# drnatebrown/col-bwt

Measured on AMD Instinct MI355X. Metric: query bases/s, higher is better.
Workload: dtype int64

## Files before the change

col-bwt_amd/csrc/fat2_query.hip:

```cpp
#include <hip/hip_runtime.h>
#include <stdint.h>

#include "device_layout.h"
#include "fat_cursor.h"
#include "fat_layout.h"
#include "lane_io.h"
#include "lane_out.h"
#include "query_kernels.h"

namespace colbwt {

namespace {

constexpr uint32_t kOffMis0 = 0xFFFFFFFCu;
constexpr uint32_t kOffMis1 = 0xFFFFFFFBu;

#ifdef COLBWT_COUNT_TRIPS
#define FAT2_STAT(k) (++stat[k])
#else
#define FAT2_STAT(k) ((void)0)
#endif

__device__ __forceinline__ uint32_t mis_slot(const uint8_t *top, uint32_t own, uint32_t c) {
    const uint32_t aidx = top[own], cidx = top[c];
    const uint32_t slot = cidx < aidx ? cidx : cidx - 1;
    return cidx < 4 && slot < kFatSlots ? slot : kFatSlots;
}

template <int K, typename PmlT, bool kDeep>
__global__ __launch_bounds__(kQueryBlock)
void fat2_query_kernel(FatTable T, const uint8_t *__restrict__ bases, const uint64_t *__restrict__ read_off,
                       uint64_t n_reads, uint32_t big_reads, uint32_t tail_permille,
                       PmlT *__restrict__ pml, uint8_t *__restrict__ cid) {
    constexpr bool kWide = sizeof(PmlT) == 4;
    __shared__ uint4 s_stage[kWaves][8][64];
    __shared__ uint4 s_win[kWaves][4][64];
    __shared__ uint32_t s_claim;
    __shared__ uint8_t s_top[256];
    const uint32_t wave = threadIdx.x >> 6, lane = threadIdx.x & 63u, g8 = lane & ~7u, p = lane & 7u;
    uint32_t *const s_jx = reinterpret_cast<uint32_t *>(&s_stage[wave][7][48]);
    ChunkPlan plan;
    plan.init(n_reads, big_reads, tail_permille);
    if (threadIdx.x == 0) s_claim = 0;
    s_top[threadIdx.x] = (uint8_t)fat_top_index(T.top4, threadIdx.x);
    __syncthreads();
    uint32_t *const claim = &s_claim;
    ReadCursor rc;
    bool done;
    rc.c_next = threadIdx.x;
    rc.request_chunk(plan, read_off);
    rc.commit();
    done = !rc.enter_chunk(plan, claim);

    OutRuns acc;
    uint32_t trip = 0;
    LaneWindow win;
    win.init(rc.off + rc.k - 1);
    uint4 (*const my_win)[64] = s_win[wave];

    uint32_t j = done ? 0u : T.r - 1;
    uint32_t o = kOffLastPos;
    uint32_t L = 0;
    const uint4 *const my_row = &s_stage[wave][p][g8];

#ifdef COLBWT_COUNT_TRIPS
    unsigned long long stat[8] = {0, 0, 0, 0, 0, 0, 0, 0};
#endif
    while (__any(!done)) {
        bool step_back = false;
        if (!done && rc.k == 0 && !rc.next_in_flight && (rc.r != rc.r_lo || rc.nc_ready)) {
            if (rc.r != rc.r_lo) {
                rc.r -= 1;
                rc.k = rc.off - rc.next_off;
                rc.off = rc.next_off;
                step_back = rc.r > rc.r_lo;
            } else if (kWide || acc.cnt == 0) {
                done = !rc.enter_chunk(plan, claim);
                if (!done) win.init(rc.off + rc.k - 1);
            }
            j = done ? 0u : T.r - 1;
            o = kOffLastPos;
            L = 0;
        }
        const bool live = !done && rc.k != 0;
        uint64_t &k = rc.k;
        const uint64_t g = rc.off + k - 1;

        s_jx[lane] = j;
        wave_sync();
        {
            const uint4 ja = *reinterpret_cast<const uint4 *>(&s_jx[g8]);
            const uint4 jb = *reinterpret_cast<const uint4 *>(&s_jx[g8 + 4]);
            const uint32_t jq[8] = {ja.x, ja.y, ja.z, ja.w, jb.x, jb.y, jb.z, jb.w};
            wave_sync();
#pragma unroll
            for (uint32_t q = 0; q < 8; ++q)
                __builtin_amdgcn_global_load_lds(T.lines + (uint64_t)jq[q] * kFatRowBytes + ((p ^ q) << 4), &s_stage[wave][q][0],
                                                 16, 0, 0);
        }
        if (live && win.avail(g) < (k < 8u ? (uint32_t)k : 8u)) win.request(my_win, bases, g);
        if (step_back) { rc.in_next = read_off[rc.r - 1]; rc.next_in_flight = true; }
        if (!done && rc.fetch_pending) rc.request_chunk(plan, read_off);
        lds_dma_landed();
        rc.commit();

        const uint32_t have = live ? win.avail(g) : 0u;
        uint32_t consumed = 0, l_new = 0, keep = 0xFFFFFFFFu, keep1 = 0xFFFFFFFFu;
        uint64_t ids = 0;
        if (!live || have == 0) FAT2_STAT(5);
        if (live && have != 0) {
            const uint64_t W = win.get8(my_win, lane, g);
            const uint32_t left = k < have ? (uint32_t)k : have;
            if (o == kOffMis0 || o == kOffMis1) {
                FAT2_STAT(2);
                const uint32_t h4 = !kDeep && o == kOffMis1 ? 4u : 0u;
                const uint4 e0 = my_row[(h4 + 0u) ^ p], e1 = my_row[(h4 + 1u) ^ p], e2 = my_row[(h4 + 2u) ^ p],
                            e3 = my_row[(h4 + 3u) ^ p];
                const uint32_t carry = L;
                const uint32_t t1 = (e0.y >> 16) & 0xFFu, d1 = e0.y >> 24, v1 = e3.z & 7u;
                uint32_t oc = 4;
                if (left >= 2) {
                    const uint32_t c2 = (uint32_t)(W >> 48) & 0xFFu;
                    const uint32_t s2 = mis_slot(s_top, t1, c2);
                    if (c2 == t1) oc = 0;
                    else if (s2 < kFatSlots && ((v1 >> s2) & 1u)) oc = 1 + s2;
                }
                if (oc < 4) {
                    const uint32_t J = oc == 0 ? e0.z : oc == 1 ? e0.w : oc == 2 ? e1.x : e1.y;
                    const uint32_t rho = oc == 0 ? e1.z : oc == 1 ? e1.w : oc == 2 ? e2.x : e2.y;
                    const uint32_t pw = oc < 2 ? e2.z : e2.w, P = (oc & 1u) ? pw >> 16 : pw & 0xFFFFu;
                    const uint32_t ch = (e3.x >> (8 * oc)) & 0xFFu, cd = (e3.y >> (8 * oc)) & 0xFFu;
                    const uint32_t vo = (e3.z >> (4 + 4 * oc)) & 7u;
                    consumed = 2;
                    l_new = 1;
                    keep = oc == 0 ? 0xFFFFFFFFu : 0u;
                    ids = (uint64_t)(d1 | (carry << 8));
                    L = oc == 0 ? 1u : 0u;
                    uint32_t nJ = J, nP = P, nrho = rho, nch = ch, ncd = cd, nv = vo, seen = 2;
                    if constexpr (kDeep) {
                        if (left >= 3 && ((uint32_t)(W >> 40) & 0xFFu) == ch) {
                            const uint4 f0 = my_row[4u ^ p], f1 = my_row[5u ^ p], f2 = my_row[6u ^ p], f3 = my_row[7u ^ p];
                            nJ = oc == 0 ? f0.x : oc == 1 ? f0.y : oc == 2 ? f0.z : f0.w;
                            nrho = oc == 0 ? f1.x : oc == 1 ? f1.y : oc == 2 ? f1.z : f1.w;
                            const uint32_t pw2 = oc < 2 ? f2.x : f2.y;
                            nP = (oc & 1u) ? pw2 >> 16 : pw2 & 0xFFFFu;
                            nch = (f2.z >> (8 * oc)) & 0xFFu;
                            ncd = (f2.w >> (8 * oc)) & 0xFFu;
                            nv = (f3.x >> (4 * oc)) & 7u;
                            consumed = 3;
                            seen = 3;
                            ids = (uint64_t)(cd | (d1 << 8) | (carry << 16));
                            if (oc == 0) { l_new = 2; keep = 0xFFFFFFFFu; }
                            else { l_new = 1; keep = 0xFFFFFFFFu; keep1 = 0u; }
                            L += 1;
                        }
                    }
                    if (k > consumed) {
                        uint32_t sn = kFatSlots;
                        if (left > seen) {
                            const uint32_t cn = (uint32_t)(W >> (8u * (7u - seen))) & 0xFFu;
                            if (cn != nch) sn = mis_slot(s_top, nch, cn);
                        }
                        if (sn < kFatSlots && ((nv >> sn) & 1u)) {
                            const uint32_t e = nrho * kFatSlots + sn;
                            j = T.slot_line0 + (kDeep ? e : e >> 1);
                            o = kDeep ? kOffMis0 : kOffMis0 - (e & 1u);
                            L = ncd;
                        } else {
                            j = nJ;
                            o = nP;
                        }
                    }
                } else {
                    consumed = 1;
                    l_new = 0;
                    ids = (uint64_t)carry;
                    L = 0;
                    j = e0.x;
                    o = e0.y & 0xFFFFu;
                }
            } else {
                FAT2_STAT(0);
                const uint4 r0 = my_row[0 ^ p];
                const uint4 r1 = my_row[1 ^ p];
                const uint64_t CH = (uint64_t)r0.x | ((uint64_t)r0.y << 32);
                const uint64_t CID = (uint64_t)r0.z | ((uint64_t)r0.w << 32);
                const uint32_t len = r1.x & 0xFFFFu;
                uint32_t skip = 0;
                bool stay = false;
                if (o == kOffPred) { o = len - 1; skip = 1; }
                else if (o == kOffSucc) { o = 0; skip = 1; }
                else if (o >= len && j < T.r - 1) {
                    o -= len;
                    j += 1;
                    stay = true;
                    FAT2_STAT(1);
                } else {
                    o = o < len ? o : len - 1;
                }
                if (!stay) {
                    const uint64_t X = skip ? ((W >> 8) ^ CH) & 0x00FFFFFFFFFFFFFFull : W ^ CH;
                    const uint32_t run = matching_top_bytes(X);
                    const uint32_t cap = left + skip < (uint32_t)K ? left + skip : (uint32_t)K;
                    uint32_t steps = run < cap ? run : cap;
                    bool own_jump = true, to_entry = false;
                    uint32_t e_next = 0, carry = 0;
                    if (run < cap) {
                        const uint32_t d = run + 1u, sh = 8u * (8u - d);
                        const uint32_t c = (uint32_t)(W >> (sh + 8u * skip)) & 0xFFu;
                        const uint32_t s = mis_slot(s_top, (uint32_t)(CH >> sh) & 0xFFu, c);
                        if (s < kFatSlots && ((r1.w >> (3u * run + s)) & 1u)) {
                            const uint32_t rho = reinterpret_cast<const uint32_t *>(&my_row[((kFatRho / 16) + (run >> 2)) ^ p])[run & 3u];
                            e_next = rho * kFatSlots + s;
                            carry = (uint32_t)(CID >> sh) & 0xFFu;
                            to_entry = true;
                            own_jump = false;
                        }
                    }
                    if (run == 0 && !to_entry) {
                        const uint32_t c = (uint32_t)(W >> 56);
                        const uint32_t cidx = T.cmap[c];
                        bool moved = false;
                        if (cidx != kAbsent) moved = fat_threshold_scan(T, j, o, c, cidx);
                        FAT2_STAT(moved ? 3 : 4);
                        if (moved) {
                            steps = 1;
                            consumed = 1;
                            l_new = 0;
                            own_jump = false;
                        } else {
                            const uint32_t st = matching_top_bytes(X & 0x00FFFFFFFFFFFFFFull);
                            const uint32_t cap0 = left < (uint32_t)K ? left : (uint32_t)K;
                            steps = st < cap0 ? st : cap0;
                            consumed = steps;
                            l_new = steps - 1;
                        }
                    } else {
                        consumed = steps - skip;
                        l_new = L + consumed;
                    }
                    L = l_new;
                    ids = steps ? CID >> (8u * (8u - steps)) : 0ull;
                    if (k == consumed) {
                    } else if (to_entry) {
                        FAT2_STAT(6);
                        j = T.slot_line0 + (kDeep ? e_next : e_next >> 1);
                        o = kDeep ? kOffMis0 : kOffMis0 - (e_next & 1u);
                        L = carry;
                    } else if (own_jump) {
                        const uint32_t e = steps - 1;
                        const uint32_t I = reinterpret_cast<const uint32_t *>(&my_row[((kFatI / 16) + (e >> 2)) ^ p])[e & 3u];
                        const uint32_t Oh = reinterpret_cast<const uint16_t *>(&my_row[((kFatO / 16) + (e >> 3)) ^ p])[e & 7u];
                        const uint64_t cuts = (uint64_t)r1.y | ((uint64_t)r1.z << 32);
                        const uint32_t cut = (uint32_t)(cuts >> (8 * e)) & 0xFFu, cut_a = cut & 0xFu, len_b = cut >> 4;
                        j = I;
                        if (cut_a != kSKCutNone && o >= cut_a) {
                            j += 1;
                            o -= cut_a;
                            if (len_b != kSKCutNone && o >= len_b) {
                                j += 1;
                                o -= len_b;
                            }
                        } else {
                            o += Oh;
                        }
                    }
                }
            }
            if constexpr (kWide) {
                for (uint32_t e = 0; e < consumed; ++e) {
                    pml[g - consumed + 1 + e] = (PmlT)((e < 2 ? keep : keep1) ? l_new - e : 0u);
                    cid[g - consumed + 1 + e] = (uint8_t)(ids >> (8 * e));
                }
            } else {
                acc.push_run(consumed, l_new, keep, keep1, (uint32_t)ids, (uint32_t)(ids >> 32));
            }
            k -= consumed;
        }
        wave_sync();
        if constexpr (!kWide) {
#ifdef COLBWT_ABL_NO_FLUSH
            if ((trip & (OutRuns::kPeriod - 1)) == OutRuns::kPeriod - 1) acc.cnt = acc.cnt > 90 ? 1 : 0;
#else
            if ((trip & (OutRuns::kPeriod - 1)) == OutRuns::kPeriod - 1)
                acc.flush_wave((uint16_t *)pml, cid, rc.off + rc.k, !done, rc.k == 0 && rc.r == rc.r_lo, &s_stage[wave][0][0], lane);
#endif
        }
        ++trip;
        wave_sync();
    }
#ifdef COLBWT_COUNT_TRIPS
    for (int q = 0; q < 8; ++q) atomicAdd(&g_fat_stats[q], stat[q]);
#endif
}

template <int K>
void launch_steps2(const FatTable &T, const uint8_t *d_bases, const uint64_t *d_read_off, uint64_t n_reads, uint64_t n_bases,
                   void *d_pml, int pml_bytes, uint8_t *d_cid, hipStream_t stream) {
    const bool deep = T.entry_shift == 7;
    if (pml_bytes == 2 && deep) launch_persistent<fat2_query_kernel<K, uint16_t, true>>(T, d_bases, d_read_off, n_reads, n_bases, (uint16_t *)d_pml, d_cid, stream);
    else if (pml_bytes == 2) launch_persistent<fat2_query_kernel<K, uint16_t, false>>(T, d_bases, d_read_off, n_reads, n_bases, (uint16_t *)d_pml, d_cid, stream);
    else if (deep) launch_persistent<fat2_query_kernel<K, uint32_t, true>>(T, d_bases, d_read_off, n_reads, n_bases, (uint32_t *)d_pml, d_cid, stream);
    else launch_persistent<fat2_query_kernel<K, uint32_t, false>>(T, d_bases, d_read_off, n_reads, n_bases, (uint32_t *)d_pml, d_cid, stream);
}

}

void launch_fat2_query(const FatTable &T, const uint8_t *d_bases, const uint64_t *d_read_off, uint64_t n_reads, uint64_t n_bases,
                       void *d_pml, int pml_bytes, uint8_t *d_cid, hipStream_t stream) {
    if (n_reads == 0) return;
#define X(K) \
    if (T.steps == K) launch_steps2<K>(T, d_bases, d_read_off, n_reads, n_bases, d_pml, pml_bytes, d_cid, stream);
    COLBWT_FAT_STEPS(X)
#undef X
}

#ifdef COLBWT_COUNT_TRIPS
extern "C" int colbwt_debug_fat2_stats(unsigned long long *out8, int reset) {
    if (hipMemcpyFromSymbol(out8, HIP_SYMBOL(g_fat_stats), 8 * sizeof(unsigned long long)) != hipSuccess) return -1;
    if (reset) {
        unsigned long long z[8] = {0, 0, 0, 0, 0, 0, 0, 0};
        if (hipMemcpyToSymbol(HIP_SYMBOL(g_fat_stats), z, sizeof(z)) != hipSuccess) return -1;
    }
    return 0;
}
#endif

}
```

col-bwt_amd/csrc/fat_build.hip:

```cpp
#include <hip/hip_runtime.h>
#include <stdint.h>

#include <functional>
#include <string>
#include <vector>

#include "../../include/colbwt.h"
#include "dev_mem.h"
#include "device_layout.h"
#include "fat_layout.h"
#include "jump_tables.h"
#include "lf_device.h"
#include "query_kernels.h"
#include "read_sampler.h"
#include "refine.h"

namespace colbwt {

namespace {

struct PlainLevel {
    const uint64_t *idx;
    const uint32_t *I;
    const uint16_t *O;
// ... 140 lines not shown
}

__global__ __launch_bounds__(256) void rho_kernel(const uint8_t *__restrict__ org, uint32_t r, uint32_t *__restrict__ rho,
                                                  uint32_t *__restrict__ rho_first) {
    const uint64_t i = (uint64_t)blockIdx.x * 256 + threadIdx.x;
    if (i >= r) return;
    const uint32_t flag = org[i] ? 1u : 0u;
    const uint32_t id = rho[i] + flag - 1u;
    rho[i] = id;
    if (flag) rho_first[id] = (uint32_t)i;
}

__global__ __launch_bounds__(256) void fat_slot_flags_kernel(PlainLevel P, FatTable T, const uint32_t *__restrict__ rho,
                                                             const uint32_t *__restrict__ rho_first, uint8_t *__restrict__ flags) {
    const uint64_t i64 = (uint64_t)blockIdx.x * 256 + threadIdx.x;
    if (i64 >= P.r) return;
    const uint32_t i = (uint32_t)i64;
    const uint32_t a_dense = T.cmap[P.meta[i] & 0xFFu];
    uint32_t f = (a_dense < 4 ? a_dense : kFatOwnOther) << 4;
    const uint32_t head = rho_first[rho[i]];
    const uint32_t top = T.sigma < 4 ? T.sigma : 4;
    for (uint32_t cidx = 0; cidx < top; ++cidx) {
        if (cidx == a_dense) continue;
        const uint32_t slot = hint_slot(cidx, a_dense);
        if (slot >= kFatSlots) continue;
        uint32_t tj, hj;
        uint64_t to, ho;
        if (!fat_slot_target(P, T, i, cidx, tj, to)) continue;
        if (head != i && (!fat_slot_target(P, T, head, cidx, hj, ho) || hj != tj || ho != to)) continue;
        f |= 1u << slot;
    }
    flags[i] = (uint8_t)f;
}

template <int K, bool kMis>
__global__ __launch_bounds__(256) void fat_pack_kernel(PlainLevel P, FatTable T, const uint32_t *__restrict__ rho,
                                                       const uint8_t *__restrict__ sflags, uint8_t *__restrict__ lines) {
    const uint64_t i64 = (uint64_t)blockIdx.x * 256 + threadIdx.x;
    if (i64 >= P.r) return;
    const uint32_t i = (uint32_t)i64;
    uint32_t w[kFatRowBytes / 4];
#pragma unroll
    for (uint32_t q = 0; q < kFatRowBytes / 4; ++q) w[q] = 0;
    const uint64_t len = P.idx[(uint64_t)i + 1] - P.idx[i];
    put_half(w, kFatLen, (uint32_t)len);

    uint32_t j = i;
    uint64_t t = 0;
    uint32_t own_ch = 0;
#pragma unroll
    for (int s = 1; s <= K; ++s) {
        const uint32_t meta = P.meta[j];
        if (s == 1) own_ch = meta & 0xFFu;
        put_byte(w, kFatCh + (8 - s), meta & 0xFFu);
        put_byte(w, kFatCid + (8 - s), meta >> 8);
        if constexpr (kMis) {
            bool one_origin = true;
            if (s == K) {
                const uint64_t end = P.idx[j] + t + len;
                for (uint64_t q = (uint64_t)j + 1; q < P.r && P.idx[q] < end; ++q) one_origin = one_origin && !P.org[q];
            }
            w[kFatRho / 4 + (s - 1)] = rho[j];
            if (one_origin) w[kFatVal / 4] |= (uint32_t)(sflags[j] & 7u) << (3 * (s - 1));
        }
        plain_lf(P, j, t);
        w[kFatI / 4 + (s - 1)] = j;
        put_half(w, kFatO + 2 * (s - 1), (uint32_t)t);
        uint32_t cut = kSKCutNone, len_b = kSKCutNone;
        if ((uint64_t)j + 1 < P.r) {
            const uint64_t c = P.idx[(uint64_t)j + 1] - P.idx[j] - t;
            if (c < kSKCutNone) {
                cut = (uint32_t)c;
                if ((uint64_t)j + 2 < P.r) {
                    const uint64_t l = P.idx[(uint64_t)j + 2] - P.idx[(uint64_t)j + 1];
                    if (l < kSKCutNone) len_b = (uint32_t)l;
                }
            }
        }
        put_byte(w, kFatCut + (s - 1), cut | (len_b << 4));
    }

    if constexpr (kMis) {
        put_byte(w, kFatFlags, sflags[i]);
    } else {
        const uint32_t a_dense = T.cmap[own_ch];
        const uint32_t aidx = a_dense < 4 ? a_dense : kFatOwnOther;
        uint32_t flags = aidx << 4;
        const uint32_t top = T.sigma < 4 ? T.sigma : 4;
        for (uint32_t cidx = 0; cidx < top; ++cidx) {
            if (cidx == a_dense) continue;
            const uint32_t slot = hint_slot(cidx, a_dense);
            if (slot >= kFatSlots) continue;
            uint32_t tj;
            uint64_t to;
            if (!fat_slot_target(P, T, i, cidx, tj, to)) continue;
            flags |= 1u << slot;
            const uint32_t sb = kFatSlot0 + slot * kFatSlotBytes;
            plain_lf(P, tj, to);
            w[sb >> 2] = tj;
            put_half(w, sb + kFatSlotP, (uint32_t)to);
            const uint32_t meta = P.meta[tj];
            put_byte(w, sb + kFatSlotCh2, meta & 0xFFu);
            put_byte(w, sb + kFatSlotCid2, meta >> 8);
            plain_lf(P, tj, to);
            w[(sb >> 2) + 1] = tj;
            put_half(w, sb + kFatSlotP + 2, (uint32_t)to);
        }
        put_byte(w, kFatFlags, flags);
    }
    uint4 *dst = reinterpret_cast<uint4 *>(lines + (uint64_t)i * kFatRowBytes);
#pragma unroll
    for (uint32_t q = 0; q < kFatRowBytes / 16; ++q) dst[q] = make_uint4(w[4 * q], w[4 * q + 1], w[4 * q + 2], w[4 * q + 3]);
}

template <bool kDeep>
__global__ __launch_bounds__(256) void fat_mis_pack_kernel(PlainLevel P, FatTable T, const uint32_t *__restrict__ rho,
                                                           const uint32_t *__restrict__ rho_first,
                                                           const uint8_t *__restrict__ sflags, uint8_t *__restrict__ entries) {
    const uint64_t e = (uint64_t)blockIdx.x * 256 + threadIdx.x;
    if (e >= (uint64_t)T.n_rho * kFatSlots) return;
    constexpr uint32_t kDwords = (kDeep ? 2 * kMisBytes : kMisBytes) / 4;
    uint32_t w[kDwords];
#pragma unroll
    for (uint32_t q = 0; q < kDwords; ++q) w[q] = 0;
    const uint32_t i = rho_first[e / kFatSlots], slot = (uint32_t)(e % kFatSlots);
    if ((sflags[i] >> slot) & 1u) {
        const uint32_t a_dense = T.cmap[P.meta[i] & 0xFFu];
        uint32_t tj;
        uint64_t to;
        fat_slot_target(P, T, i, slot < a_dense ? slot : slot + 1, tj, to);
        plain_lf(P, tj, to);
        const uint32_t J1 = tj;
        const uint64_t P1 = to;
        const uint32_t m1 = P.meta[J1], a1 = T.cmap[m1 & 0xFFu], v1 = sflags[J1] & 7u;
        w[kMisJ1] = J1;
        w[kMisP1] = (uint32_t)P1 | ((m1 & 0xFFu) << 16) | ((m1 >> 8) << 24);
        w[kMisVal] = v1;
        for (uint32_t o = 0; o < 4; ++o) {
            uint32_t j = J1;
            uint64_t t = P1;
            if (o) {
                if (!((v1 >> (o - 1)) & 1u)) continue;
                fat_slot_target(P, T, J1, (o - 1) < a1 ? o - 1 : o, j, t);
            }
            plain_lf(P, j, t);
            const uint32_t m = P.meta[j];
            w[kMisJ + o] = j;
            w[kMisRho + o] = rho[j];
            put_half(w, 4 * kMisP + 2 * o, (uint32_t)t);
            put_byte(w, 4 * kMisCh + o, m & 0xFFu);
            put_byte(w, 4 * kMisCid + o, m >> 8);
            w[kMisVal] |= (uint32_t)(sflags[j] & 7u) << (4 + 4 * o);
            if constexpr (kDeep) {
                plain_lf(P, j, t);
                const uint32_t m2 = P.meta[j];
                w[kMisDeep + kMisJ - 2 + o] = j;
                w[kMisDeep + kMisRho - 2 + o] = rho[j];
                put_half(w, 4 * (kMisDeep + kMisP - 2) + 2 * o, (uint32_t)t);
                put_byte(w, 4 * (kMisDeep + kMisCh - 2) + o, m2 & 0xFFu);
                put_byte(w, 4 * (kMisDeep + kMisCid - 2) + o, m2 >> 8);
                w[kMisDeep + kMisVal - 2] |= (uint32_t)(sflags[j] & 7u) << (4 * o);
            }
        }
    }
    uint4 *dst = reinterpret_cast<uint4 *>(entries + e * (kDwords * 4));
#pragma unroll
    for (uint32_t q = 0; q < kDwords / 4; ++q) dst[q] = make_uint4(w[4 * q], w[4 * q + 1], w[4 * q + 2], w[4 * q + 3]);
}

template <class Src>
int refine_plain(const Src &S, uint64_t src_rows, uint64_t n, PlainLevel &out, PlainBuffers &buf, std::string &err) {
    DevPtr first, park;
    uint64_t total = 0;
    {
        const int rc = count_and_scan(S, src_rows, first, total, err);
        if (rc != COLBWT_OK) return rc;
    }
    if (total > 0xFFFFFFFEull) {
        err = "line-row layout needs " + std::to_string(total) + " rows at one of its levels (> 2^32-2)";
        return COLBWT_ERR_NOMEM;
    }
    if (total * kFatRowBytes > dev_available_bytes()) {
        if (getenv("COLBWT_ALLOC_LOG"))
            fprintf(stderr, "[colbwt alloc] ? %llu rows x 128 bytes = %.2f GB against %.2f GB available\n", (unsigned long long)total,
                    total * 128e-9, dev_available_bytes() * 1e-9);
        err = "line-row layout: " + std::to_string(total) + " rows at a refinement level need more HBM than is available";
        return COLBWT_ERR_NOMEM;
    }
    const uint32_t r_new = (uint32_t)total;
    SK_TRY(buf.idx.alloc(((uint64_t)r_new + 2) * sizeof(uint64_t)));
    SK_TRY(buf.I.alloc(((uint64_t)r_new + 1) * sizeof(uint32_t)));
    SK_TRY(buf.O.alloc(((uint64_t)r_new + 1) * sizeof(uint16_t)));
    SK_TRY(buf.meta.alloc(((uint64_t)r_new + 1) * sizeof(uint16_t)));
    SK_TRY(buf.thr.alloc(((uint64_t)r_new + 1) * sizeof(uint64_t)));
    SK_TRY(buf.org.alloc((uint64_t)r_new + 1));
    SK_TRY(park.alloc(((uint64_t)r_new + 1) * sizeof(uint64_t)));
    uint64_t *const d_idx = buf.idx.as<uint64_t>(), *const d_thr = buf.thr.as<uint64_t>(), *const d_park = park.as<uint64_t>();
    uint32_t *const d_I = buf.I.as<uint32_t>(), *const d_first = first.as<uint32_t>();
    uint16_t *const d_O = buf.O.as<uint16_t>(), *const d_meta = buf.meta.as<uint16_t>();
    uint8_t *const d_org = buf.org.as<uint8_t>();
    const uint32_t rblocks = (uint32_t)((src_rows + 255) / 256);
    hipLaunchKernelGGL(plain_emit_kernel<Src>, dim3(rblocks), dim3(256), 0, 0, S, (const uint32_t *)d_first, d_idx, d_I, d_meta,
                       d_thr, d_org, d_park, r_new);
    SK_TRY(hipGetLastError());
    SK_TRY(hipStreamSynchronize(0));
    const uint32_t nblocks = (uint32_t)(((uint64_t)r_new + 255) / 256);
    hipLaunchKernelGGL(plain_link_kernel, dim3(nblocks), dim3(256), 0, 0, (const uint32_t *)d_first, (const uint64_t *)d_idx,
                       (const uint64_t *)d_park, d_I, d_O, r_new);
    SK_TRY(hipGetLastError());
    SK_TRY(hipStreamSynchronize(0));
    out.idx = d_idx;
    out.I = d_I;
    out.O = d_O;
    out.meta = d_meta;
    out.thr = d_thr;
    out.org = d_org;
    out.n = n;
    out.r = r_new;
    return COLBWT_OK;
}

constexpr uint64_t kDeepReserve = 32ull << 30;

template <int K>
int build_fat_steps(const DevTable &T1, const HintChars &chars, int mismatch_lines, FatTable &out, FatBuffers &buf, std::string &err,
                    const std::function<void()> &source_done, int &failed_level) {
    failed_level = 2;
    const uint8_t *cmap = T1.cmap;
    const uint32_t sigma = T1.sigma;
    PlainLevel cur{};
    PlainBuffers cur_buf;
    LoadClock clock;
    {
        const SrcL1 s1{T1, chars};
        const int rc = refine_plain(s1, T1.r, T1.n, cur, cur_buf, err);
        if (rc != COLBWT_OK) return rc;
    }
    clock.lap("  refinement level 2");
    source_done();
    clock.lap("  one-step tables freed");
    for (int level = 3; level <= K; ++level) {
        failed_level = level;
        PlainLevel next{};
        PlainBuffers next_buf;
        const SrcPlain sp{cur};
        const int rc = refine_plain(sp, cur.r, cur.n, next, next_buf, err);
        if (rc != COLBWT_OK) return rc;
        cur_buf.release();
        cur = next;
        cur_buf.idx = std::move(next_buf.idx);
        cur_buf.I = std::move(next_buf.I);
        cur_buf.O = std::move(next_buf.O);
        cur_buf.meta = std::move(next_buf.meta);
        cur_buf.thr = std::move(next_buf.thr);
        cur_buf.org = std::move(next_buf.org);
        clock.lap("  refinement level (3..K)");
    }

    failed_level = K + 1;
    const uint32_t r = cur.r;
    out = FatTable{};
    out.n = cur.n;
    out.r = r;
    out.sigma = sigma;
    out.cmap = cmap;
    out.nblk = (uint32_t)(((uint64_t)r + (1u << kBlockShift) - 1) >> kBlockShift);
    out.steps = K;
    out.top4 = 0;
    for (uint32_t k = 0; k < 4; ++k) out.top4 |= (uint32_t)chars.c[k < sigma ? k : 0] << (8 * k);

    SK_TRY(buf.chr.alloc((uint64_t)r + 64));
    uint8_t *const d_chr = buf.chr.as<uint8_t>();
    const uint32_t nblocks = (uint32_t)(((uint64_t)r + 255) / 256);
    hipLaunchKernelGGL(plain_chars_kernel, dim3(nblocks), dim3(256), 0, 0, cur.meta, r, d_chr);
    SK_TRY(hipGetLastError());
    const uint64_t entries = (uint64_t)out.nblk * sigma;
    SK_TRY(buf.next.alloc((entries ? entries : 1) * sizeof(uint32_t)));
    SK_TRY(buf.prev.alloc((entries ? entries : 1) * sizeof(uint32_t)));
    uint32_t *const d_next = buf.next.as<uint32_t>(), *const d_prev = buf.prev.as<uint32_t>();
    hipLaunchKernelGGL(chr_block_first_last_kernel, dim3((out.nblk + 3) / 4), dim3(256), 0, 0, (const uint8_t *)d_chr, r, out.nblk,
                       sigma, cmap, d_next, d_prev);
    SK_TRY(hipGetLastError());
    SK_TRY(hipStreamSynchronize(0));
    {
        std::vector<uint32_t> first(entries), last(entries), next, prev;
        SK_TRY(hipMemcpy(first.data(), d_next, entries * sizeof(uint32_t), hipMemcpyDeviceToHost));
        SK_TRY(hipMemcpy(last.data(), d_prev, entries * sizeof(uint32_t), hipMemcpyDeviceToHost));
        finish_jump_tables(first, last, out.nblk, sigma, next, prev);
        SK_TRY(hipMemcpy(d_next, next.data(), entries * sizeof(uint32_t), hipMemcpyHostToDevice));
        SK_TRY(hipMemcpy(d_prev, prev.data(), entries * sizeof(uint32_t), hipMemcpyHostToDevice));
    }
    out.chr = d_chr;
    out.next_tbl = d_next;
    out.prev_tbl = d_prev;
    out.idx = cur.idx;
    out.thr = cur.thr;

    clock.lap("  characters, jump tables");
    DevPtr rho_buf, rho_first_buf, sflags_buf;
    uint64_t mis_lines = 0;
    uint32_t *d_rho = nullptr, *d_rho_first = nullptr;
    uint8_t *d_sflags = nullptr;
    if (mismatch_lines) {
        SK_TRY(rho_buf.alloc(((uint64_t)r + 1) * sizeof(uint32_t)));
        d_rho = rho_buf.as<uint32_t>();
        const uint8_t *const d_org = cur.org;
        hipLaunchKernelGGL(org_flags_kernel, dim3(nblocks), dim3(256), 0, 0, d_org, r, d_rho);
        SK_TRY(hipGetLastError());
        uint64_t n_rho = 0;
        {
            const int rc = exclusive_scan_u32(d_rho, r, n_rho, err);
            if (rc != COLBWT_OK) return rc;
        }
        if (mismatch_lines == 3) {
// ... 130 lines not shown
```

col-bwt_amd/csrc/fat_layout.h:

```cpp
#pragma once
#include <hip/hip_runtime.h>
#include <stdint.h>

#include "device_layout.h"

namespace colbwt {

#define COLBWT_FAT_STEPS(X) X(4) X(5) X(6) X(7) X(8)

constexpr uint32_t kFatRowBytes = 128;
constexpr uint32_t kFatSlots = 3;
constexpr uint32_t kFatSlotSteps = 2;
constexpr uint32_t kFatOwnOther = 7;
constexpr uint32_t kFatCh = 0, kFatCid = 8, kFatLen = 16, kFatFlags = 18, kFatCut = 20, kFatI = 32, kFatO = 64,
                   kFatSlot0 = 80, kFatSlotBytes = 16;
constexpr uint32_t kFatSlotP = 8, kFatSlotCh2 = 12, kFatSlotCid2 = 13;
constexpr uint32_t kFatVal = 28, kFatRho = 80;
constexpr uint32_t kMisBytes = 64, kMisJ1 = 0, kMisP1 = 1, kMisJ = 2, kMisRho = 6, kMisP = 10, kMisCh = 12, kMisCid = 13, kMisVal = 14;
constexpr uint32_t kMisDeep = 16;

struct FatTable {
    const uint8_t *lines;
    const uint8_t *chr;
    const uint64_t *idx;
    const uint64_t *thr;
    const uint32_t *next_tbl;
    const uint32_t *prev_tbl;
    const uint8_t *cmap;
    uint64_t n;
    uint32_t r;
    uint32_t sigma;
    uint32_t nblk;
    uint32_t steps;
    uint32_t top4;
    uint32_t slot_line0;
    uint32_t n_rho;
    uint32_t entry_shift;
};

__device__ __forceinline__ uint32_t fat_byte(const uint32_t *w, uint32_t off) { return (w[off >> 2] >> (8 * (off & 3u))) & 0xFFu; }
__device__ __forceinline__ uint32_t fat_half(const uint32_t *w, uint32_t off) { return (w[off >> 2] >> (8 * (off & 2u))) & 0xFFFFu; }

__device__ __forceinline__ uint32_t fat_top_index(uint32_t top4, uint32_t c) {
    uint32_t x = 4;
    x = ((top4 >> 24) & 0xFFu) == c ? 3u : x;
    x = ((top4 >> 16) & 0xFFu) == c ? 2u : x;
    x = ((top4 >> 8) & 0xFFu) == c ? 1u : x;
    x = (top4 & 0xFFu) == c ? 0u : x;
    return x;
}

__device__ __forceinline__ uint32_t fat_succ_char(const FatTable &T, uint32_t i, uint32_t c, uint32_t cidx) {
    const uint32_t blk = i >> kBlockShift;
    const uint64_t lim = (((uint64_t)blk + 1) << kBlockShift);
    const uint64_t end = lim < T.r ? lim : T.r;
    for (uint64_t s = (uint64_t)i + 1; s < end; ++s)
        if (T.chr[s] == c) return (uint32_t)s;
    if (blk + 1 < T.nblk) return T.next_tbl[(uint64_t)(blk + 1) * T.sigma + cidx];
    return kNone;
}
__device__ __forceinline__ uint32_t fat_pred_char(const FatTable &T, uint32_t i, uint32_t c, uint32_t cidx) {
    const uint32_t blk = i >> kBlockShift;
    const uint32_t first = blk << kBlockShift;
    for (uint32_t q = i; q > first;) {
        --q;
        if (T.chr[q] == c) return q;
    }
    if (blk > 0) return T.prev_tbl[(uint64_t)blk * T.sigma + cidx];
    return kNone;
}

}
```

col-bwt_amd/csrc/lane_out.h:

```cpp
#pragma once
#include <hip/hip_runtime.h>
#include <stdint.h>

#include "lane_io.h"

#ifdef COLBWT_ABL_NO_STORES
#define COLBWT_ABL_IF if (ltop == 0xFFFFFFF1u)
#else
#define COLBWT_ABL_IF
#endif

namespace colbwt {

struct OutRuns {
    static constexpr uint32_t kBlock = 64;
    static constexpr uint32_t kPeriod = 4;
    static constexpr uint32_t kSlotQ = 6, kItemQ = 4;
    static constexpr uint32_t lds_q(uint32_t slots) { return slots * kSlotQ + 2 * slots * kItemQ; }

    uint32_t z0a = 0, z0b = 0, z0c = 0, z1a = 0, z1b = 0, z1c = 0;
    uint32_t ltop = 0;
    uint32_t c0 = 0, c1 = 0, c2 = 0, c3 = 0, c4 = 0, c5 = 0, c6 = 0, c7 = 0, c8 = 0, c9 = 0, c10 = 0, c11 = 0, c12 = 0, c13 = 0, c14 = 0, c15 = 0, c16 = 0, c17 = 0, c18 = 0, c19 = 0, c20 = 0, c21 = 0, c22 = 0, c23 = 0;
    uint32_t cnt = 0;

    __device__ __forceinline__ void push_run(uint32_t n, uint32_t l_new, uint32_t keep, uint32_t keep1, uint32_t ids_lo,
                                             uint32_t ids_hi) {
        const uint32_t in_run = (1u << n) - 1u;
        uint32_t p0 = l_new < n ? 1u << l_new : 0u;
        p0 |= (keep ? 0u : 3u) & in_run;
        p0 |= (keep1 ? 0u : 0xCu) & in_run;
        const uint32_t top = (1u << n) >> 1;
        const uint32_t p1 = (keep & keep1) != 0u && l_new == n ? top : 0u;
        z0c = (uint32_t)(((((uint64_t)z0c << 32) | z0b) << n) >> 32);
        z0b = (uint32_t)(((((uint64_t)z0b << 32) | z0a) << n) >> 32);
        z0a = (z0a << n) | p0;
        z1c = (uint32_t)(((((uint64_t)z1c << 32) | z1b) << n) >> 32);
        z1b = (uint32_t)(((((uint64_t)z1b << 32) | z1a) << n) >> 32);
        z1a = (z1a << n) | p1;
        const bool d4 = n & 8u, d2 = n & 4u;
        c23 = d4 ? c21 : c23;
        c22 = d4 ? c20 : c22;
        c21 = d4 ? c19 : c21;
        c20 = d4 ? c18 : c20;
        c19 = d4 ? c17 : c19;
        c18 = d4 ? c16 : c18;
        c17 = d4 ? c15 : c17;
        c16 = d4 ? c14 : c16;
        c15 = d4 ? c13 : c15;
        c14 = d4 ? c12 : c14;
        c13 = d4 ? c11 : c13;
        c12 = d4 ? c10 : c12;
        c11 = d4 ? c9 : c11;
        c10 = d4 ? c8 : c10;
        c9 = d4 ? c7 : c9;
        c8 = d4 ? c6 : c8;
        c7 = d4 ? c5 : c7;
        c6 = d4 ? c4 : c6;
        c5 = d4 ? c3 : c5;
        c4 = d4 ? c2 : c4;
        c3 = d4 ? c1 : c3;
        c2 = d4 ? c0 : c2;
        c1 = d4 ? 0u : c1;
        c0 = d4 ? 0u : c0;
        c23 = d2 ? c22 : c23;
        c22 = d2 ? c21 : c22;
        c21 = d2 ? c20 : c21;
        c20 = d2 ? c19 : c20;
        c19 = d2 ? c18 : c19;
        c18 = d2 ? c17 : c18;
        c17 = d2 ? c16 : c17;
        c16 = d2 ? c15 : c16;
        c15 = d2 ? c14 : c15;
        c14 = d2 ? c13 : c14;
        c13 = d2 ? c12 : c13;
        c12 = d2 ? c11 : c12;
        c11 = d2 ? c10 : c11;
        c10 = d2 ? c9 : c10;
        c9 = d2 ? c8 : c9;
        c8 = d2 ? c7 : c8;
        c7 = d2 ? c6 : c7;
        c6 = d2 ? c5 : c6;
        c5 = d2 ? c4 : c5;
        c4 = d2 ? c3 : c4;
        c3 = d2 ? c2 : c3;
        c2 = d2 ? c1 : c2;
        c1 = d2 ? c0 : c1;
        c0 = d2 ? 0u : c0;
        const uint32_t sel8 = 0x07060504u - 0x01010101u * (n & 3u);
        c23 = __builtin_amdgcn_perm(c23, c22, sel8);
        c22 = __builtin_amdgcn_perm(c22, c21, sel8);
        c21 = __builtin_amdgcn_perm(c21, c20, sel8);
        c20 = __builtin_amdgcn_perm(c20, c19, sel8);
        c19 = __builtin_amdgcn_perm(c19, c18, sel8);
        c18 = __builtin_amdgcn_perm(c18, c17, sel8);
        c17 = __builtin_amdgcn_perm(c17, c16, sel8);
        c16 = __builtin_amdgcn_perm(c16, c15, sel8);
        c15 = __builtin_amdgcn_perm(c15, c14, sel8);
        c14 = __builtin_amdgcn_perm(c14, c13, sel8);
        c13 = __builtin_amdgcn_perm(c13, c12, sel8);
        c12 = __builtin_amdgcn_perm(c12, c11, sel8);
        c11 = __builtin_amdgcn_perm(c11, c10, sel8);
        c10 = __builtin_amdgcn_perm(c10, c9, sel8);
        c9 = __builtin_amdgcn_perm(c9, c8, sel8);
        c8 = __builtin_amdgcn_perm(c8, c7, sel8);
        c7 = __builtin_amdgcn_perm(c7, c6, sel8);
        c6 = __builtin_amdgcn_perm(c6, c5, sel8);
        c5 = __builtin_amdgcn_perm(c5, c4, sel8);
        c4 = __builtin_amdgcn_perm(c4, c3, sel8);
        c3 = __builtin_amdgcn_perm(c3, c2, sel8);
        c2 = __builtin_amdgcn_perm(c2, c1, sel8);
        c1 = __builtin_amdgcn_perm(c1, c0, sel8);
        c0 = __builtin_amdgcn_perm(c0, 0u, sel8);
        const uint32_t mlo = n >= 4 ? 0xFFFFFFFFu : (1u << (8 * n)) - 1u;
        const uint32_t mhi = n >= 8 ? 0xFFFFFFFFu : (n > 4 ? (1u << (8 * (n - 4))) - 1u : 0u);
        c0 |= ids_lo & mlo;
        c1 |= ids_hi & mhi;
        cnt += n;
    }

    static __device__ __forceinline__ void shr96(uint64_t &lo, uint32_t &hi, uint32_t s) {
        if (s >= 64) {
            lo = (uint64_t)(hi >> (s - 64));
            hi = 0;
        } else if (s) {
            lo = (lo >> s) | ((uint64_t)hi << (64 - s));
            hi = s < 32 ? hi >> s : 0u;
        }
    }
    static __device__ __forceinline__ uint64_t low64_from(uint32_t a, uint32_t b, uint32_t c, uint32_t s) {
        uint64_t lo = ((uint64_t)b << 32) | a;
        uint32_t hi = c;
        shr96(lo, hi, s);
        return lo;
    }
    __device__ __forceinline__ uint32_t park_item(uint4 *item, uint32_t slot, uint32_t e_lo, uint32_t count, uint64_t addr, uint32_t lt) const {
        const uint32_t o_lo = (uint32_t)addr & (kBlock - 1), o_hi = o_lo + count;
        const uint64_t in_item = count >= 64 ? ~0ull : (1ull << count) - 1ull;
        const uint64_t Z0 = (low64_from(z0a, z0b, z0c, e_lo) & in_item) << o_lo;
        const uint64_t Z1 = (low64_from(z1a, z1b, z1c, e_lo) & in_item) << o_lo;
        const uint32_t z0w[2] = {(uint32_t)Z0, (uint32_t)(Z0 >> 32)}, z1w[2] = {(uint32_t)Z1, (uint32_t)(Z1 >> 32)};
        uint32_t pm[8];
        uint32_t v = lt;
#pragma unroll
        for (int p = 7; p >= 0; --p) {
            const uint32_t b0 = (z0w[p >> 2] >> (8 * (p & 3))) & 0xFFu, b1 = (z1w[p >> 2] >> (8 * (p & 3))) & 0xFFu;
            pm[p] = (v & 0xFFFFu) | (b0 << 16) | (b1 << 24);
            const uint32_t lo_p = o_lo > 8u * p ? o_lo : 8u * p, hi_p = o_hi < 8u * p + 8u ? o_hi : 8u * p + 8u;
            if (hi_p > lo_p) {
                const uint32_t bits = b0 | b1;
                if (bits) {
                    const uint32_t q = (uint32_t)__builtin_ctz(bits);
                    v = q - (lo_p - 8u * p) + ((b1 >> q) & 1u);
                } else {
                    v += hi_p - lo_p;
                }
            }
        }
        item[0] = make_uint4(slot, e_lo, count, (uint32_t)addr);
        item[1] = make_uint4((uint32_t)(addr >> 32), 0u, 0u, 0u);
        item[2] = make_uint4(pm[0], pm[1], pm[2], pm[3]);
        item[3] = make_uint4(pm[4], pm[5], pm[6], pm[7]);
        return v;
    }

    template <uint32_t kSlots = 32>
    __device__ __forceinline__ void flush_wave(uint16_t *pml, uint8_t *cid, uint64_t gl, bool active, bool final, uint4 *lds,
                                               uint32_t lane) {
        constexpr uint32_t kItemBase = kSlots * kSlotQ;
        const uint32_t below = (0u - (uint32_t)gl) & (kBlock - 1);
        const bool has_a = active && below < cnt;
        const uint32_t rest = below < cnt ? below : cnt;
        const bool has_b = active && final && rest != 0;
        const unsigned long long emit = __ballot(has_a || has_b);
        if (emit == 0) return;
        const uint32_t n_a = has_a ? cnt - below : 0u;
        uint32_t v_cut = ltop;
        const unsigned long long lt = (1ull << lane) - 1ull;
        const uint32_t rank = (uint32_t)__builtin_popcountll(emit & lt), lanes = (uint32_t)__builtin_popcountll(emit);
        for (uint32_t first = 0; first < lanes; first += kSlots) {
            const bool mine = (has_a || has_b) && rank >= first && rank < first + kSlots;
            const bool rag_a = mine && has_a && n_a != kBlock, rag_b = mine && has_b, full_a = mine && has_a && n_a == kBlock;
            const unsigned long long m_ra = __ballot(rag_a), m_rb = __ballot(rag_b), m_fa = __ballot(full_a);
            const uint32_t n_ra = (uint32_t)__builtin_popcountll(m_ra), n_rb = (uint32_t)__builtin_popcountll(m_rb);
            const uint32_t n_rag = n_ra + n_rb, n_items = n_rag + (uint32_t)__builtin_popcountll(m_fa);
            if (mine) {
// ... 109 lines not shown
```

Before: 149.0 billion.

## Repack deep mismatch rows into generic slots including a mismatch-after-match case

```diff
diff --git a/col-bwt_amd/csrc/fat2_query.hip b/col-bwt_amd/csrc/fat2_query.hip
--- a/col-bwt_amd/csrc/fat2_query.hip
+++ b/col-bwt_amd/csrc/fat2_query.hip
@@ -105,7 +105,7 @@
         rc.commit();
 
         const uint32_t have = live ? win.avail(g) : 0u;
-        uint32_t consumed = 0, l_new = 0, keep = 0xFFFFFFFFu, keep1 = 0xFFFFFFFFu;
+        uint32_t consumed = 0, l_new = 0, keep = 0xFFFFFFFFu, keep1 = 0xFFFFFFFFu, zero0 = 0;
         uint64_t ids = 0;
         if (!live || have == 0) FAT2_STAT(5);
         if (live && have != 0) {
@@ -137,27 +137,47 @@
                     ids = (uint64_t)(d1 | (carry << 8));
                     L = oc == 0 ? 1u : 0u;
                     uint32_t nJ = J, nP = P, nrho = rho, nch = ch, ncd = cd, nv = vo, seen = 2;
+                    uint32_t sn = kFatSlots;
+                    bool looked = false;
                     if constexpr (kDeep) {
-                        if (left >= 3 && ((uint32_t)(W >> 40) & 0xFFu) == ch) {
-                            const uint4 f0 = my_row[4u ^ p], f1 = my_row[5u ^ p], f2 = my_row[6u ^ p], f3 = my_row[7u ^ p];
-                            nJ = oc == 0 ? f0.x : oc == 1 ? f0.y : oc == 2 ? f0.z : f0.w;
-                            nrho = oc == 0 ? f1.x : oc == 1 ? f1.y : oc == 2 ? f1.z : f1.w;
-                            const uint32_t pw2 = oc < 2 ? f2.x : f2.y;
-                            nP = (oc & 1u) ? pw2 >> 16 : pw2 & 0xFFFFu;
-                            nch = (f2.z >> (8 * oc)) & 0xFFu;
-                            ncd = (f2.w >> (8 * oc)) & 0xFFu;
-                            nv = (f3.x >> (4 * oc)) & 7u;
-                            consumed = 3;
-                            seen = 3;
-                            ids = (uint64_t)(cd | (d1 << 8) | (carry << 16));
-                            if (oc == 0) { l_new = 2; keep = 0xFFFFFFFFu; }
-                            else { l_new = 1; keep = 0xFFFFFFFFu; keep1 = 0u; }
-                            L += 1;
+                        if (left >= 3) {
+                            const uint32_t c3 = (uint32_t)(W >> 40) & 0xFFu;
+                            uint32_t kind = 0;
+                            if (c3 != ch) {
+                                sn = mis_slot(s_top, ch, c3);
+                                kind = sn < kFatSlots && ((vo >> sn) & 1u) ? 1u + sn : 4u;
+                            }
+                            looked = true;
+                            const uint32_t t = kind < 4u ? (uint32_t)(kDeepSlotLut >> (16u * oc + 4u * kind)) & 0xFu : kDeepNone;
+                            if (t < kDeepSlots) {
+                                const uint32_t dw = kDeepSlot0 + kDeepSlotDwords * t;
+                                nJ = reinterpret_cast<const uint32_t *>(&my_row[(dw >> 2) ^ p])[dw & 3u];
+                                nrho = reinterpret_cast<const uint32_t *>(&my_row[((dw + 1u) >> 2) ^ p])[(dw + 1u) & 3u];
+                                const uint32_t x = reinterpret_cast<const uint32_t *>(&my_row[((dw + 2u) >> 2) ^ p])[(dw + 2u) & 3u];
+                                nP = x & 0xFFFFu;
+                                nch = (x >> 16) & 0xFFu;
+                                ncd = x >> 24;
+                                nv = (e3.w >> (3u * t)) & 7u;
+                                consumed = 3;
+                                seen = 3;
+                                looked = false;
+                                sn = kFatSlots;
+                                ids = (uint64_t)(cd | (d1 << 8) | (carry << 16));
+                                if (kind == 0) {
+                                    if (oc == 0) { l_new = 2; keep = 0xFFFFFFFFu; }
+                                    else { l_new = 1; keep = 0xFFFFFFFFu; keep1 = 0u; }
+                                    L += 1;
+                                } else {
+                                    FAT2_STAT(7);
+                                    if (oc == 0) { l_new = 2; zero0 = 1u; }
+                                    else keep1 = 0u;
+                                    L = 0;
+                                }
+                            }
                         }
                     }
                     if (k > consumed) {
-                        uint32_t sn = kFatSlots;
-                        if (left > seen) {
+                        if (!looked && left > seen) {
                             const uint32_t cn = (uint32_t)(W >> (8u * (7u - seen))) & 0xFFu;
                             if (cn != nch) sn = mis_slot(s_top, nch, cn);
                         }
@@ -269,11 +289,11 @@
             }
             if constexpr (kWide) {
                 for (uint32_t e = 0; e < consumed; ++e) {
-                    pml[g - consumed + 1 + e] = (PmlT)((e < 2 ? keep : keep1) ? l_new - e : 0u);
+                    pml[g - consumed + 1 + e] = (PmlT)((e < 2 ? keep : keep1) && !(e == 0 && zero0) ? l_new - e : 0u);
                     cid[g - consumed + 1 + e] = (uint8_t)(ids >> (8 * e));
                 }
             } else {
-                acc.push_run(consumed, l_new, keep, keep1, (uint32_t)ids, (uint32_t)(ids >> 32));
+                acc.template push_run<kDeep>(consumed, l_new, keep, keep1, (uint32_t)ids, (uint32_t)(ids >> 32), zero0);
             }
             k -= consumed;
         }
diff --git a/col-bwt_amd/csrc/fat_build.hip b/col-bwt_amd/csrc/fat_build.hip
--- a/col-bwt_amd/csrc/fat_build.hip
+++ b/col-bwt_amd/csrc/fat_build.hip
@@ -316,14 +316,23 @@
             put_byte(w, 4 * kMisCid + o, m >> 8);
             w[kMisVal] |= (uint32_t)(sflags[j] & 7u) << (4 + 4 * o);
             if constexpr (kDeep) {
-                plain_lf(P, j, t);
-                const uint32_t m2 = P.meta[j];
-                w[kMisDeep + kMisJ - 2 + o] = j;
-                w[kMisDeep + kMisRho - 2 + o] = rho[j];
-                put_half(w, 4 * (kMisDeep + kMisP - 2) + 2 * o, (uint32_t)t);
-                put_byte(w, 4 * (kMisDeep + kMisCh - 2) + o, m2 & 0xFFu);
-                put_byte(w, 4 * (kMisDeep + kMisCid - 2) + o, m2 >> 8);
-                w[kMisDeep + kMisVal - 2] |= (uint32_t)(sflags[j] & 7u) << (4 * o);
+                const uint32_t a = T.cmap[m & 0xFFu], v = sflags[j] & 7u;
+#pragma unroll
+                for (uint32_t q = 0; q < kDeepSlots; ++q) {
+                    if (kDeepSlot[q].outcome != o) continue;
+                    uint32_t j3 = j;
+                    uint64_t t3 = t;
+                    if (const uint32_t kind = kDeepSlot[q].kind) {
+                        if (!((v >> (kind - 1)) & 1u)) continue;
+                        fat_slot_target(P, T, j, (kind - 1) < a ? kind - 1 : kind, j3, t3);
+                    }
+                    plain_lf(P, j3, t3);
+                    const uint32_t m3 = P.meta[j3];
+                    w[kDeepSlot0 + kDeepSlotDwords * q] = j3;
+                    w[kDeepSlot0 + kDeepSlotDwords * q + 1] = rho[j3];
+                    w[kDeepSlot0 + kDeepSlotDwords * q + 2] = ((uint32_t)t3 & 0xFFFFu) | ((m3 & 0xFFu) << 16) | ((m3 >> 8) << 24);
+                    w[kDeepVal] |= (uint32_t)(sflags[j3] & 7u) << (3 * q);
+                }
             }
         }
     }
diff --git a/col-bwt_amd/csrc/fat_layout.h b/col-bwt_amd/csrc/fat_layout.h
--- a/col-bwt_amd/csrc/fat_layout.h
+++ b/col-bwt_amd/csrc/fat_layout.h
@@ -17,7 +17,21 @@
 constexpr uint32_t kFatSlotP = 8, kFatSlotCh2 = 12, kFatSlotCid2 = 13;
 constexpr uint32_t kFatVal = 28, kFatRho = 80;
 constexpr uint32_t kMisBytes = 64, kMisJ1 = 0, kMisP1 = 1, kMisJ = 2, kMisRho = 6, kMisP = 10, kMisCh = 12, kMisCid = 13, kMisVal = 14;
-constexpr uint32_t kMisDeep = 16;
+constexpr uint32_t kDeepVal = 15, kDeepSlot0 = 16, kDeepSlotDwords = 3, kDeepSlots = 5, kDeepNone = 15;
+struct DeepSlot {
+    uint8_t outcome;
+    uint8_t kind;
+};
+constexpr DeepSlot kDeepSlot[kDeepSlots] = {{0, 0}, {1, 0}, {2, 0}, {3, 0}, {0, 1}};
+constexpr uint64_t deep_slot_lut() {
+    uint64_t lut = ~0ull;
+    for (uint32_t t = 0; t < kDeepSlots; ++t) {
+        const uint32_t sh = 4u * (4u * kDeepSlot[t].outcome + kDeepSlot[t].kind);
+        lut = (lut & ~(0xFull << sh)) | ((uint64_t)t << sh);
+    }
+    return lut;
+}
+constexpr uint64_t kDeepSlotLut = deep_slot_lut();
 
 struct FatTable {
     const uint8_t *lines;
diff --git a/col-bwt_amd/csrc/lane_out.h b/col-bwt_amd/csrc/lane_out.h
--- a/col-bwt_amd/csrc/lane_out.h
+++ b/col-bwt_amd/csrc/lane_out.h
@@ -23,14 +23,19 @@
     uint32_t c0 = 0, c1 = 0, c2 = 0, c3 = 0, c4 = 0, c5 = 0, c6 = 0, c7 = 0, c8 = 0, c9 = 0, c10 = 0, c11 = 0, c12 = 0, c13 = 0, c14 = 0, c15 = 0, c16 = 0, c17 = 0, c18 = 0, c19 = 0, c20 = 0, c21 = 0, c22 = 0, c23 = 0;
     uint32_t cnt = 0;
 
+    template <bool kZero = false>
     __device__ __forceinline__ void push_run(uint32_t n, uint32_t l_new, uint32_t keep, uint32_t keep1, uint32_t ids_lo,
-                                             uint32_t ids_hi) {
+                                             uint32_t ids_hi, uint32_t zero = 0u) {
         const uint32_t in_run = (1u << n) - 1u;
         uint32_t p0 = l_new < n ? 1u << l_new : 0u;
         p0 |= (keep ? 0u : 3u) & in_run;
         p0 |= (keep1 ? 0u : 0xCu) & in_run;
         const uint32_t top = (1u << n) >> 1;
-        const uint32_t p1 = (keep & keep1) != 0u && l_new == n ? top : 0u;
+        uint32_t p1 = (keep & keep1) != 0u && l_new == n ? top : 0u;
+        if constexpr (kZero) {
+            p0 |= zero & in_run;
+            p1 &= ~zero;
+        }
         z0c = (uint32_t)(((((uint64_t)z0c << 32) | z0b) << n) >> 32);
         z0b = (uint32_t)(((((uint64_t)z0b << 32) | z0a) << n) >> 32);
         z0a = (z0a << n) | p0;
```

Result: slower. 138.9 billion (-6.8%).
